# vvvwo/KSS-ICP

Hardware: AMD Instinct MI355X
Metric: icp_iterations_per_sec (higher is better)
Workload: dtype f32; 1 GPU; C2: one 100000x100000 uniform-sphere pair per GPU, 50 fixed ICP iterations + fitness pass per step (exact NN + cov reduce + host 3x3 SVD), R_z(10deg), jitter 1e-3; n_src=100000, n_tgt=100000, pairs_per_gpu=1, nn_engine=cell list + brute-force fallback, nn_arithmetic=reference (no fma)

## Files before the change

kss-icp_amd/csrc/kss_device.hpp:

```cpp
#pragma once
#include <hip/hip_runtime.h>

#include "kss_internal.hpp"

namespace kss {

template <bool FMA>
__device__ __forceinline__ float dist2(float sx, float sy, float sz, float tx, float ty, float tz) {
    const float dx = sx - tx, dy = sy - ty, dz = sz - tz;
    if constexpr (FMA) {
        return __builtin_fmaf(dx, dx, __builtin_fmaf(dy, dy, dz * dz));
    } else {
        return (dx * dx + dy * dy) + dz * dz;
    }
}

__device__ __forceinline__ int cell_coord(float v, float o, float inv_h, int g) {
    int c = (int)floorf((v - o) * inv_h);
    c = c < 0 ? 0 : c;
    return c >= g ? g - 1 : c;
}

__device__ __forceinline__ double wave_sum(double v) {
#pragma unroll
// ... 110 lines not shown
    v = 0.0;
    if (threadIdx.x < NSUMS)
        for (int gg = 0; gg < G; ++gg) v += shg[gg][threadIdx.x];
    return *s_ok != 0;
}

__device__ __forceinline__ void pub_put(unsigned long long* pub, int64_t slot, double v, unsigned long long seq, unsigned torn_xor = 0u) {
    const unsigned long long b = (unsigned long long)__double_as_longlong(v);
    u32x4 o;
    o.x = (unsigned)b; o.y = (unsigned)(b >> 32); o.z = (unsigned)seq; o.w = kss_mix3(o.x, o.y, o.z);
    o.x ^= torn_xor;
    unsigned long long* dst = pub + 2 * slot;
    asm volatile("global_store_dwordx4 %0, %1, off sc0 sc1" ::"v"(dst), "v"(o) : "memory");
}

constexpr int PASS_BS = 512;
constexpr int PASS_FG = PASS_BS / NSUMS;

template <typename F>
__device__ __forceinline__ double dpp_f64(double x, F f) {
    const int lo = f(__double2loint(x)), hi = f(__double2hiint(x));
    return __hiloint2double(hi, lo);
}
__device__ __forceinline__ double xor8(double x) { return dpp_f64(x, [](int v) { return __builtin_amdgcn_mov_dpp(v, 0x128, 0xf, 0xf, false); }); }
__device__ __forceinline__ double xor4(double x) {
    return dpp_f64(x, [](int v) {
        int r = __builtin_amdgcn_mov_dpp(v, 0x104, 0xf, 0x5, false);
        return __builtin_amdgcn_update_dpp(r, v, 0x114, 0xf, 0xa, false);
    });
}
__device__ __forceinline__ double xor2(double x) { return dpp_f64(x, [](int v) { return __builtin_amdgcn_mov_dpp(v, 0x4e, 0xf, 0xf, false); }); }
__device__ __forceinline__ double xor1(double x) { return dpp_f64(x, [](int v) { return __builtin_amdgcn_mov_dpp(v, 0xb1, 0xf, 0xf, false); }); }

__device__ __forceinline__ double level32(double a, double b) {
    unsigned alo = (unsigned)__double2loint(a), ahi = (unsigned)__double2hiint(a), blo = (unsigned)__double2loint(b), bhi = (unsigned)__double2hiint(b);
    asm volatile("s_nop 1\n\tv_permlane32_swap_b32 %0, %1\n\ts_nop 1" : "+v"(alo), "+v"(blo));
    asm volatile("s_nop 1\n\tv_permlane32_swap_b32 %0, %1\n\ts_nop 1" : "+v"(ahi), "+v"(bhi));
    return __hiloint2double((int)ahi, (int)alo) + __hiloint2double((int)bhi, (int)blo);
}
__device__ __forceinline__ double level16(double a, double b) {
    unsigned alo = (unsigned)__double2loint(a), ahi = (unsigned)__double2hiint(a), blo = (unsigned)__double2loint(b), bhi = (unsigned)__double2hiint(b);
    asm volatile("s_nop 1\n\tv_permlane16_swap_b32 %0, %1\n\ts_nop 1" : "+v"(alo), "+v"(blo));
    asm volatile("s_nop 1\n\tv_permlane16_swap_b32 %0, %1\n\ts_nop 1" : "+v"(ahi), "+v"(bhi));
    return __hiloint2double((int)ahi, (int)alo) + __hiloint2double((int)bhi, (int)blo);
}
__device__ __forceinline__ double tree_low4(double x) {
    x += xor8(x); x += xor4(x); x += xor2(x); x += xor1(x);
    return x;
}

__device__ __forceinline__ void wave_tree16(double (&v)[16]) {
#pragma unroll
    for (int j = 0; j < 8; ++j) v[j] = level32(v[j], v[j + 8]);
#pragma unroll
    for (int j = 0; j < 4; ++j) v[j] = level16(v[j], v[j + 4]);
#pragma unroll
    for (int j = 0; j < 4; ++j) v[j] = tree_low4(v[j]);
}
__device__ __forceinline__ double wave_tree2(double a, double b) {
    double x = level32(a, b);
    x = level16(x, x);
    return tree_low4(x);
}

__device__ __forceinline__ void accumulate_corr(double (&acc)[NSUMS], float px, float py, float pz,
                                                float qx, float qy, float qz, float d2f, double max_d2) {
    const double d2 = (double)d2f;
    acc[17] += d2;
    acc[18] += sqrt(d2);
    if (!(d2 > max_d2)) {
        const double p[3] = {(double)px, (double)py, (double)pz};
        const double q[3] = {(double)qx, (double)qy, (double)qz};
        acc[0] += 1.0;
#pragma unroll
        for (int k = 0; k < 3; ++k) { acc[1 + k] += p[k]; acc[4 + k] += q[k]; }
#pragma unroll
        for (int k = 0; k < 3; ++k)
#pragma unroll
            for (int l = 0; l < 3; ++l) acc[7 + 3 * k + l] += p[k] * q[l];
        acc[16] += d2;
    }
}


}
```

kss-icp_amd/csrc/kss_grid.hip:

```cpp
#pragma clang fp contract(off)

#include <hip/hip_runtime.h>

#include <cstring>

#include <rocprim/rocprim.hpp>

#include <cstdlib>

#include "kss_internal.hpp"
#include "kss_device.hpp"

namespace kss {

__global__ __launch_bounds__(256) void grid_count2_kernel(const float4* __restrict__ tgt, int nt, int nbt, const float4* __restrict__ src, int ns,
                                                          GridParams gp, int32_t* __restrict__ counts, int32_t* __restrict__ slot) {
    const bool is_src = (int)blockIdx.x >= nbt;
    const int i = ((int)blockIdx.x - (is_src ? nbt : 0)) * 256 + (int)threadIdx.x;
    if (i >= (is_src ? ns : nt)) return;
    const float4 p = is_src ? src[i] : tgt[i];
    const int cx = cell_coord(p.x, gp.ox, gp.inv_h, gp.gx), cy = cell_coord(p.y, gp.oy, gp.inv_h, gp.gy),
              cz = cell_coord(p.z, gp.oz, gp.inv_h, gp.gz);
    slot[(is_src ? nt : 0) + i] = atomicAdd(&counts[(is_src ? gp.gx * gp.gy * gp.gz : 0) + (cz * gp.gy + cy) * gp.gx + cx], 1);
}
// ... 294 lines not shown
        if (t == 4) continue;
        const float g2 = ey2[t % 3] + ez2[t / 3];
        const bool need = ok[t] && !(rho < g2 * 0.999999f);
        const bool left = !(rho < (g2 + exl2) * 0.999999f), right = !(rho < (g2 + exr2) * 0.999999f);
        const int lo = left ? s0[t] : s1[t];
        const int hi = right ? s3[t] : s2[t];
        const bool take = need && hi > lo;
        rowq[min(nrow, 7)][threadIdx.x] = make_int2(lo, hi);
        nrow += take ? 1 : 0;
        total += take ? hi - lo : 0;
    }
    int cur = 0, end = 0, nxt = 0;
    if (nrow > 0) { const int2 v = rowq[0][threadIdx.x]; cur = v.x; end = v.y; nxt = 1; }
    for (int e = 0; e < total; e += U) {
        int at[U];
#pragma unroll
        for (int j = 0; j < U; ++j) {
            at[j] = min(cur, end - 1);
            ++cur;
            if (cur >= end && nxt < nrow) { const int2 v = rowq[nxt][threadIdx.x]; cur = v.x; end = v.y; ++nxt; }
        }
        float4 pt[U];
#pragma unroll
        for (int j = 0; j < U; ++j) pt[j] = sorted[at[j]];
#pragma unroll
        for (int j = 0; j < U; ++j) {
            const unsigned long long kk = point_key<FMA>(pt[j], qx, qy, qz);
            if (kk < key) { key = kk; kpos = at[j]; }
            const float dd = e + j < total ? __uint_as_float((unsigned)(kk >> 32)) : __builtin_inff();
            m2 = __builtin_amdgcn_fmed3f(m1, m2, dd);
            m1 = fminf(m1, dd);
        }
    }
    return n4 + total;
}

__device__ __forceinline__ void row_range(const GridParams& gp, const int32_t* __restrict__ cell_start, float qx, float qy, float qz,
                                          int cx, int cy, int cz, float rho, int t, int& lo, int& hi) {
    lo = hi = 0;
    const int tz = t / 3, ty = t - 3 * tz;
    const int z = cz + tz - 1, y = cy + ty - 1;
    if (!(t >= 0 && t < 9 && z >= 0 && z < gp.gz && y >= 0 && y < gp.gy)) return;
    const int4u v = *(const int4u*)(cell_start + (z * gp.gy + y) * gp.gx + cx - 1);
    const int s0 = cx > 0 ? v.x : v.y, s1 = v.y, s2 = v.z, s3 = cx + 1 < gp.gx ? v.w : v.z;
    const float exl = fmaxf((qx - (gp.ox + (float)cx * gp.h)) - gp.eps, 0.f), exr = fmaxf(((gp.ox + (float)(cx + 1) * gp.h) - qx) - gp.eps, 0.f);
    const float eyl = fmaxf((qy - (gp.oy + (float)cy * gp.h)) - gp.eps, 0.f), eyr = fmaxf(((gp.oy + (float)(cy + 1) * gp.h) - qy) - gp.eps, 0.f);
    const float ezl = fmaxf((qz - (gp.oz + (float)cz * gp.h)) - gp.eps, 0.f), ezr = fmaxf(((gp.oz + (float)(cz + 1) * gp.h) - qz) - gp.eps, 0.f);
    const float ey2 = ty == 0 ? eyl * eyl : ty == 2 ? eyr * eyr : 0.f, ez2 = tz == 0 ? ezl * ezl : tz == 2 ? ezr * ezr : 0.f;
    const float g2 = ey2 + ez2;
    if (rho < g2 * 0.999999f) return;
    const bool left = !(rho < (g2 + exl * exl) * 0.999999f), right = !(rho < (g2 + exr * exr) * 0.999999f);
    lo = left ? s0 : s1;
    hi = right ? s3 : s2;
    if (hi < lo) hi = lo;
}

template <bool FMA, int U, bool TWO>
__device__ __forceinline__ void row_walk(const GridParams& gp, const int32_t* __restrict__ cell_start, const float4* __restrict__ sorted,
                                         float qx, float qy, float qz, int cx, int cy, int cz, float rho, int t0, int t1,
                                         unsigned long long& key, int& kpos, float& m1, float& m2) {
    m1 = __builtin_inff();
    m2 = __builtin_inff();
    int lo0, hi0, lo1 = 0, hi1 = 0;
    row_range(gp, cell_start, qx, qy, qz, cx, cy, cz, rho, t0, lo0, hi0);
    if constexpr (TWO) row_range(gp, cell_start, qx, qy, qz, cx, cy, cz, rho, t1, lo1, hi1);
    const int n0 = hi0 - lo0, total = n0 + (hi1 - lo1);
    const int last = hi1 > lo1 ? hi1 - 1 : hi0 - 1;
    for (int e = 0; e < total; e += U) {
        int at[U];
        float4 pt[U];
#pragma unroll
        for (int j = 0; j < U; ++j) {
            const int f = e + j;
            if constexpr (TWO) at[j] = f >= total ? last : f < n0 ? lo0 + f : lo1 + (f - n0);
            else at[j] = min(lo0 + f, hi0 - 1);
        }
#pragma unroll
        for (int j = 0; j < U; ++j) pt[j] = sorted[at[j]];
#pragma unroll
        for (int j = 0; j < U; ++j) {
            const unsigned long long kk = point_key<FMA>(pt[j], qx, qy, qz);
            if (kk < key) { key = kk; kpos = at[j]; }
            const float dd = e + j < total ? __uint_as_float((unsigned)(kk >> 32)) : __builtin_inff();
            m2 = __builtin_amdgcn_fmed3f(m1, m2, dd);
            m1 = fminf(m1, dd);
        }
    }
}

__global__ __launch_bounds__(256) void grid_rank_fix_kernel(const float4* __restrict__ tmp, int n, GridParams gp,
                                                            const int32_t* __restrict__ start , int shift,
                                                            float4* __restrict__ out) {
    const int j = blockIdx.x * blockDim.x + threadIdx.x;
    if (j >= n) return;
    const float4 p = tmp[j];
    const int cx = cell_coord(p.x, gp.ox, gp.inv_h, gp.gx), cy = cell_coord(p.y, gp.oy, gp.inv_h, gp.gy),
              cz = cell_coord(p.z, gp.oz, gp.inv_h, gp.gz);
    const int c = (cz * gp.gy + cy) * gp.gx + cx;
    const int lo = start[c] - shift, hi = start[c + 1] - shift;
    const int me = __float_as_int(p.w);
    int rank = 0;
    for (int k = lo; k < hi; ++k) rank += __float_as_int(tmp[k].w) < me ? 1 : 0;
    out[lo + rank] = p;
}

void launch_grid_build_pair(hipStream_t st, const float4* d_tgt, int nt, float4* d_src, int ns, const GridParams& gp, int32_t* d_counts,
                            int32_t* d_slot, int32_t* d_start, int32_t* d_block_sums, float4* d_sorted, float4* d_tmp) {
    const int ncells = gp.gx * gp.gy * gp.gz;
    const int nbt = (nt + 255) / 256, nbs = (ns + 255) / 256;
    hipLaunchKernelGGL(grid_count2_kernel, dim3(nbt + nbs), dim3(256), 0, st, d_tgt, nt, nbt, (const float4*)d_src, ns, gp, d_counts, d_slot);
    launch_scan(st, d_counts, 2 * ncells, d_start, d_block_sums, true);
    hipLaunchKernelGGL(grid_scatter2_kernel, dim3(nbt + nbs), dim3(256), 0, st, d_tgt, nt, nbt, (const float4*)d_src, ns, gp, (const int32_t*)d_slot,
                       (const int32_t*)d_start, d_sorted, d_tmp);
    hipLaunchKernelGGL(grid_rank_fix_kernel, dim3(nbs), dim3(256), 0, st, (const float4*)d_tmp, ns, gp, (const int32_t*)d_start + ncells, nt,
                       d_src);
}

struct SkipOut {
    unsigned long long key;
    int kpos;
    float rho;
    float acc;
    bool walker;
};
template <bool FMA>
__device__ __forceinline__ SkipOut skip_test(bool qok, float qx, float qy, float qz, float pold_x, float pold_y, float pold_z, const float4& prevp,
                                             const float2& st, bool chained_k, float skin_frac, float h) {
    SkipOut o;
    o.key = ~0ull; o.kpos = -1; o.rho = __builtin_inff(); o.acc = 0.f; o.walker = false;
    if (!qok) return o;
    o.walker = true;
    if (__float_as_uint(prevp.w) != ~0u) {
        o.key = point_key<FMA>(prevp, qx, qy, qz);
        o.kpos = -2;
        const float d0 = __uint_as_float((unsigned)(o.key >> 32));
        const float mx = qx - pold_x, my = qy - pold_y, mz = qz - pold_z;
        const float moved = __builtin_amdgcn_sqrtf((mx * mx + my * my) + mz * mz);
        const float acc = (st.y + moved) * 1.00001f;
        const float room = st.x - acc;
        if (chained_k && skin_frac >= 0.f && room > 1e-7f && (room * room) * 0.99999f > d0) {
            o.walker = false;
            o.acc = acc;
        } else {
            const float skin = fmaxf(skin_frac, 0.f) * h, grown = __builtin_amdgcn_sqrtf(d0) + skin;
            o.rho = !chained_k || moved * 4.f <= skin ? fmaxf(d0, grown * grown) : d0;
        }
    }
    return o;
}

template <bool FULL>
__device__ __forceinline__ void wave_row(bool have, bool kept, bool fell_back, float qx, float qy, float qz, const float4& win, double d2d, double* shw_row) {
    const int lane = threadIdx.x & 63;
    double col[16];
    {
        const double px = kept ? (double)qx : 0.0, py = kept ? (double)qy : 0.0, pz = kept ? (double)qz : 0.0;
        const double tx = kept ? (double)win.x : 0.0, ty = kept ? (double)win.y : 0.0, tz = kept ? (double)win.z : 0.0;
        col[0] = px; col[1] = py; col[2] = pz; col[3] = tx; col[4] = ty; col[5] = tz;
        col[6] = px * tx; col[7] = px * ty; col[8] = px * tz;
        col[9] = py * tx; col[10] = py * ty; col[11] = py * tz;
        col[12] = pz * tx; col[13] = pz * ty; col[14] = pz * tz;
        col[15] = kept ? d2d : 0.0;
    }
    wave_tree16(col);
    const unsigned long long mk = __builtin_amdgcn_ballot_w64(kept), mf = __builtin_amdgcn_ballot_w64(fell_back);
    double extra = 0.0;
    if constexpr (FULL) extra = wave_tree2(d2d, have ? sqrt(d2d) : 0.0);
    if ((lane & 15) == 0) {
        const int q = lane >> 4;
#pragma unroll
        for (int j = 0; j < 4; ++j) shw_row[1 + 4 * q + j] = col[j];
        if (lane == 0) {
            shw_row[0] = (double)__builtin_popcountll(mk);
            shw_row[NSUMS - 1] = (double)__builtin_popcountll(mf);
            shw_row[17] = extra;
        }
        if (lane == 32) shw_row[18] = extra;
    }
}

template <bool FMA, bool BATCH, int WQ, int NT, int U, bool FIRST = false>
__device__ __forceinline__ void serve_walkers(const PassArgs& a, const GridPairDev& pr, const int32_t* __restrict__ cs,
                                              const float4* __restrict__ sorted, int w, int nwalk, int2 (*rowq)[WQ],
                                              unsigned (*s_ent)[PASS_BS], const unsigned short* s_wl) {
#define KSS_STAMP(k) do { if (a.stamps && threadIdx.x == 0) a.stamps[(size_t)blockIdx.x * 16 + (k)] = __builtin_amdgcn_s_memrealtime(); } while (0)
    enum { WK_X, WK_Y, WK_Z, WK_IDX, WK_D2, WK_R, WK_POS, WK_FL = WK_POS, WK_COLS };
    const GridParams& gp = pr.gp;
    const int lane = threadIdx.x & 63;
    const bool row16 = 16 * nwalk <= NT, row8 = BATCH && !row16 && 8 * nwalk <= NT, rows = row16 || row8;
    const int L = row16 ? 16 : row8 ? 8 : 4 * nwalk <= WQ ? 4 : 1;
    const int nserve = rows ? NT : (WQ < NT ? WQ : NT);
    for (int rb = 0; rb < nwalk; rb += nserve / L)
    if ((int)threadIdx.x < nserve && (int)(threadIdx.x & ~63u) < (nwalk - rb) * L) {
        const int sub = (int)threadIdx.x & (L - 1);
        const int wj = rb + (L == 16 ? (int)threadIdx.x >> 4 : L == 8 ? (int)threadIdx.x >> 3 : L == 4 ? (int)threadIdx.x >> 2 : (int)threadIdx.x);
        const bool wk = wj < nwalk;
        const unsigned rowmask = L == 1 ? 0x1ffu : sub == 0 ? 0x105u : sub == 1 ? 0x050u : sub == 2 ? 0x082u : 0x028u;
        float wx = 0.f, wy = 0.f, wz = 0.f, wrho = __builtin_inff(), bnew = 0.f;
        unsigned long long wkey = ~0ull;
        int wpos = -1, owner = 0, evl = 0, rfin = 0;
        bool done = true, wfell = false;
        if (wk) {
            owner = (int)s_wl[wj];
            wx = __uint_as_float(s_ent[WK_X][owner]); wy = __uint_as_float(s_ent[WK_Y][owner]); wz = __uint_as_float(s_ent[WK_Z][owner]);
            wkey = ((unsigned long long)s_ent[WK_D2][owner] << 32) | (unsigned long long)s_ent[WK_IDX][owner];
            wpos = (int)s_ent[WK_POS][owner];
            wrho = __uint_as_float(s_ent[WK_R][owner]);
            done = false;
        }
        if (wk) {
            const int cx = cell_coord(wx, gp.ox, gp.inv_h, gp.gx), cy = cell_coord(wy, gp.oy, gp.inv_h, gp.gy),
                      cz = cell_coord(wz, gp.oz, gp.inv_h, gp.gz);
            KSS_STAMP(5);
            float m1, m2;
            if (row16) row_walk<FMA, U, false>(gp, cs, sorted, wx, wy, wz, cx, cy, cz, wrho, sub < 9 ? sub : -1, -1, wkey, wpos, m1, m2);
            else if (BATCH && row8) row_walk<FMA, U, true>(gp, cs, sorted, wx, wy, wz, cx, cy, cz, wrho, sub, sub == 0 ? 8 : -1, wkey, wpos, m1, m2);
            else if (FIRST && L == 1) evl = block_walk_first<FMA, WQ, U>(gp, cs, sorted, wx, wy, wz, cx, cy, cz, wrho, a.skin, rowq, wkey, wpos, m1, m2);
            else evl = block_walk<FMA, WQ, U>(gp, cs, sorted, wx, wy, wz, cx, cy, cz, wrho, rowmask, rowq, wkey, wpos, m1, m2);
            if (L > 1) {
#define KSS_GROUP_MERGE(X)                                                                                                          \
do {                                                                                                                            \
    const unsigned olo = (unsigned)X((int)(unsigned)wkey), ohi = (unsigned)X((int)(unsigned)(wkey >> 32));                      \
    const int opos = X(wpos);                                                                                                   \
    const float o1 = __int_as_float(X(__float_as_int(m1))), o2 = __int_as_float(X(__float_as_int(m2)));                         \
    const unsigned long long okey = ((unsigned long long)ohi << 32) | olo;                                                      \
    if (okey < wkey) { wkey = okey; wpos = opos; }                                                                            \
    m2 = fminf(fmaxf(m1, o1), fminf(m2, o2));                                \
    m1 = fminf(m1, o1);                                                                                                         \
} while (0)
                auto x1 = [](int v) { return __builtin_amdgcn_update_dpp(0, v, 0xb1, 0xf, 0xf, false); };
                auto x2 = [](int v) { return __builtin_amdgcn_update_dpp(0, v, 0x4e, 0xf, 0xf, false); };
                auto x4 = [](int v) { const int r = __builtin_amdgcn_update_dpp(v, v, 0x104, 0xf, 0x5, false); return __builtin_amdgcn_update_dpp(r, v, 0x114, 0xf, 0xa, false); };
                auto x8 = [](int v) { return __builtin_amdgcn_update_dpp(0, v, 0x128, 0xf, 0xf, false); };
                KSS_GROUP_MERGE(x1);
                KSS_GROUP_MERGE(x2);
                if (L >= 8) KSS_GROUP_MERGE(x4);
                if (L == 16) KSS_GROUP_MERGE(x8);
#undef KSS_GROUP_MERGE
            }
            float face2 = __builtin_inff();
            for (int r = 1; r <= gp.rcap; ++r) {
                if (r > 1) {
                    const int wd = 2 * r + 1;
                    const int x0 = max(cx - r, 0), x1 = min(cx + r, gp.gx - 1);
                    for (int t = 0; t < wd * wd; ++t) {
                        const int dz = t / wd - r, dy = t % wd - r;
                        const int z = cz + dz, y = cy + dy;
                        if (z < 0 || z >= gp.gz || y < 0 || y >= gp.gy) continue;
                        const int row = (z * gp.gy + y) * gp.gx;
                        if (dz == -r || dz == r || dy == -r || dy == r) {
                            scan_range<FMA>(sorted, cs[row + x0], cs[row + x1 + 1], wx, wy, wz, wkey, wpos);
                        } else {
                            if (cx - r >= 0) scan_range<FMA>(sorted, cs[row + cx - r], cs[row + cx - r + 1], wx, wy, wz, wkey, wpos);
                            if (cx + r < gp.gx) scan_range<FMA>(sorted, cs[row + cx + r], cs[row + cx + r + 1], wx, wy, wz, wkey, wpos);
                        }
                    }
                }
                const float best = __uint_as_float((unsigned)(wkey >> 32));
                float b = __builtin_inff();
                if (cx - r > 0) b = fminf(b, wx - (gp.ox + (float)(cx - r) * gp.h));
                if (cx + r < gp.gx - 1) b = fminf(b, (gp.ox + (float)(cx + r + 1) * gp.h) - wx);
                if (cy - r > 0) b = fminf(b, wy - (gp.oy + (float)(cy - r) * gp.h));
                if (cy + r < gp.gy - 1) b = fminf(b, (gp.oy + (float)(cy + r + 1) * gp.h) - wy);
                if (cz - r > 0) b = fminf(b, wz - (gp.oz + (float)(cz - r) * gp.h));
                if (cz + r < gp.gz - 1) b = fminf(b, (gp.oz + (float)(cz + r + 1) * gp.h) - wz);
                const float bs = b - gp.eps;
                if (b == __builtin_inff()) done = true;
                else if (bs > 0.f && best < bs * bs * 0.999999f) { done = true; face2 = bs * bs; }
                if (done) { rfin = r; break; }
            }
            if (done && rfin == 1 && wkey != ~0ull)
                bnew = fminf(__builtin_amdgcn_sqrtf(fminf(fminf(m2, wrho), face2) * 0.99999f) * 0.999999f, 1e30f);
        }
        if constexpr (BATCH) {
            if (__builtin_amdgcn_ballot_w64(!done) != 0ull) {
                const float4* __restrict__ tp = a.tgt4 + pr.tgt_base;
                for (int j = 0; j < pr.tgt_n; ++j) {
                    const float4 q = tp[j];
                    const float dx = wx - q.x, dy = wy - q.y, dz = wz - q.z;
                    float d;
                    if constexpr (FMA) d = __builtin_fmaf(dx, dx, __builtin_fmaf(dy, dy, dz * dz));
                    else d = (dx * dx + dy * dy) + dz * dz;
                    const unsigned long long kk = ((unsigned long long)__float_as_uint(d) << 32) | (unsigned long long)(unsigned)j;
                    if (!done && kk < wkey) { wkey = kk; wpos = -1; }
                }
                wfell = !done;
                done = true;
            }
        }
        if (wk && sub == 0) {
            bool whave = false;
            float4 ww = make_float4(0.f, 0.f, 0.f, 0.f);
            const int io = pr.src_base + (w - pr.row_base) * PASS_BS + owner;
            if (done) {
                whave = wkey != ~0ull;
                if (whave) ww = wpos >= 0 ? sorted[wpos] : wpos == -2 ? a.nn_win[io] : a.tgt4[pr.tgt_base + (int)(unsigned)(wkey & 0xffffffffull)];
            } else {
                a.keys[io] = ~0ull;
                const int ls = atomicAdd(a.list_count, 1);
                a.list[ls] = io;
                wfell = true;
            }
            a.nn_win[io] = make_float4(ww.x, ww.y, ww.z, __uint_as_float(whave ? (unsigned)wkey : ~0u));
            a.nn_state[io] = make_float2(wfell ? 0.f : bnew, 0.f);
            s_ent[WK_X][owner] = __float_as_uint(ww.x); s_ent[WK_Y][owner] = __float_as_uint(ww.y); s_ent[WK_Z][owner] = __float_as_uint(ww.z);
            s_ent[WK_IDX][owner] = (unsigned)wkey; s_ent[WK_D2][owner] = (unsigned)(wkey >> 32);
            s_ent[WK_FL][owner] = (whave ? 1u : 0u) | (wfell ? 2u : 0u);
            s_ent[WK_R][owner] = __float_as_uint(wfell ? 0.f : bnew);
        }
        KSS_STAMP(8);
        if (a.stamps) {
            int evs = evl, mx = evl;
#pragma unroll
            for (int m = 32; m > 0; m >>= 1) { evs += __shfl_xor(evs, m, 64); mx = max(mx, __shfl_xor(mx, m, 64)); }
            if (lane == 0) {
                atomicAdd(&a.stamps[(size_t)blockIdx.x * 16 + 10], (unsigned long long)evs);
                atomicAdd(&a.stamps[(size_t)blockIdx.x * 16 + 11], (unsigned long long)(((mx + 7) / 8) * 8 * 64));
            }
        }
    }
#undef KSS_STAMP
}

#ifndef KSS_BATCH_WAVES
#define KSS_BATCH_WAVES 6
#endif
#ifndef KSS_SINGLE_WAVES
#define KSS_SINGLE_WAVES 1
#endif
template <bool FMA, bool FULL, bool BATCH, bool SEARCH, bool CHAIN, bool FIRST = false>
__global__ __launch_bounds__(PASS_BS, BATCH ? KSS_BATCH_WAVES : KSS_SINGLE_WAVES) void grid_pass_kernel(const PassArgs a) {
    static_assert(!CHAIN || (!BATCH && SEARCH), "chained launches: single pair, search passes");
    static_assert(!FIRST || (!BATCH && SEARCH && !CHAIN), "the first pass: single pair, a plain search launch");
#define KSS_STAMP(k) do { if (a.stamps && threadIdx.x == 0) a.stamps[(size_t)blockIdx.x * 16 + (k)] = __builtin_amdgcn_s_memrealtime(); } while (0)
    KSS_STAMP(0);
    constexpr int BS = PASS_BS;
    const int per_xcd = (int)gridDim.x / 8;
    const int w = ((int)blockIdx.x % 8) * per_xcd + (int)blockIdx.x / 8;
    if (w >= a.total_rows) return;
    int pi = 0;
    if constexpr (BATCH) pi = a.row_pair[w];
    const GridPairDev pr = BATCH ? a.pairs[pi] : a.pair0;
    PairState ps = a.ps0;
    if constexpr (BATCH) {
        ps = a.state[pi];
        if (!ps.active) return;
    }
    const GridParams& gp = pr.gp;
    const int32_t* __restrict__ cs = a.cell_start + pr.cell_base;
    const float4* __restrict__ sorted = a.sorted;
    constexpr int WQ = FIRST ? BS : 256;
    __shared__ int2 rowq[9][WQ];
    __shared__ double shw[BS / 64][NSUMS];
    __shared__ int s_last;
    __shared__ int sh_ps[16];
    __shared__ int s_nwalk;
    __shared__ unsigned s_ent[7][BS];
    __shared__ unsigned short s_wl[BS];
    enum { WK_X, WK_Y, WK_Z, WK_IDX, WK_D2, WK_R, WK_POS, WK_FL = WK_POS, WK_COLS };
    static_assert(sizeof(PairState) == 64, "the gated launch reads the transform record as 16 dwords");
    double (*shf)[NSUMS] = reinterpret_cast<double (*)[NSUMS]>(&rowq[0][0]);
    static_assert(sizeof(double) * PASS_FG * NSUMS <= sizeof(int2) * 9 * WQ, "shf must fit inside rowq");

    const int local = (w - pr.row_base) * BS + (int)threadIdx.x;
    const bool valid = local < pr.src_n;
    const int i = pr.src_base + local;
    const int lane = threadIdx.x & 63, wave = threadIdx.x >> 6;
    bool have = false, fell_back = false;
    float qx = 0.f, qy = 0.f, qz = 0.f, d2 = 0.f;
    float4 win = make_float4(0.f, 0.f, 0.f, 0.f);
    float4 p = make_float4(0.f, 0.f, 0.f, 0.f), prevp = make_float4(0.f, 0.f, 0.f, __uint_as_float(~0u));
    float2 st = make_float2(0.f, 0.f);
    if (valid) {
        p = SEARCH ? a.src_in[i] : a.src_out[i];
        if (!SEARCH || a.use_prev) { prevp = a.nn_win[i]; st = a.nn_state[i]; }
    }
    for (int step = 0;; ++step) {
    const bool last_step = !CHAIN || step + 1 >= a.chain_len;
    const unsigned long long seq_k = a.seq + (unsigned long long)step;
    const int gate_k = a.gate_seq != 0 ? a.gate_seq + step : 0;
    unsigned int* const gate_ptr = a.gate_dev + 32 * ((a.gate_slot + step) & 1);
    float4* const src_out_k = (step & 1) ? a.src_alt : a.src_out;
    const bool last_known = a.chained == 2 && ps.pad[0] > 0;
    const bool chained_k = step > 0 || a.chained == 1 || last_known;
    const bool has_prev = __float_as_uint(prevp.w) != ~0u;
    if constexpr (SEARCH) {
        __syncthreads();
        if (threadIdx.x == 0) s_nwalk = 0;
        __syncthreads();
    }
    KSS_STAMP(13);
    if constexpr (!BATCH && SEARCH) {
        if (gate_k != 0) {
            typedef unsigned int u32x4 __attribute__((ext_vector_type(4)));
            if (a.state && w == 0 && threadIdx.x < 16) {
                const int* w32 = reinterpret_cast<const int*>(a.state);
                int v = 0, n = 0;
                bool ok = true;
                for (;;) {
                    v = __hip_atomic_load(w32 + threadIdx.x, __ATOMIC_RELAXED, __HIP_MEMORY_SCOPE_SYSTEM);
                    if (__shfl(v, 15, 64) == gate_k) break;
                    __builtin_amdgcn_s_sleep(1);
                    if (++n > a.gate_polls / 2) { ok = false; break; }
                }
                if (ok) {
                    const int g = threadIdx.x;
                    const int w0 = __shfl(v, min(3 * g, 15), 64), w1 = __shfl(v, min(3 * g + 1, 15), 64), w2 = __shfl(v, min(3 * g + 2, 15), 64);
                    if (g < 5) {
                        u32x4 o;
                        o.x = (unsigned)w0; o.y = (unsigned)w1; o.z = (unsigned)w2; o.w = (unsigned)gate_k + kss_mix3(o.x, o.y, o.z);
                        unsigned int* dst = gate_ptr + 4 * g;
                        asm volatile("global_store_dwordx4 %0, %1, off sc1" ::"v"(dst), "v"(o) : "memory");
                    }
                }
            }
            if (threadIdx.x < 8) {
// ... 3 lines not shown
                bool ok = true;
                for (;;) {
                    asm volatile("global_load_dwordx4 %0, %1, off sc0 sc1\n\ts_waitcnt vmcnt(0)" : "=&v"(v) : "v"(src) : "memory");
                    if (__builtin_amdgcn_ballot_w64(v.w - kss_mix3(v.x, v.y, v.z) == (unsigned)gate_k) == 0xffull) break;
                    __builtin_amdgcn_s_sleep(1);
                    if (++n > a.gate_polls) { ok = false; break; }
                }
                if (threadIdx.x < 5) { sh_ps[3 * threadIdx.x] = (int)v.x; sh_ps[3 * threadIdx.x + 1] = (int)v.y; sh_ps[3 * threadIdx.x + 2] = (int)v.z; }
                if (threadIdx.x == 0) { sh_ps[15] = gate_k; s_last = ok ? 1 : 0; }
            }
            __syncthreads();
            if (!s_last) return;
            int* d32 = reinterpret_cast<int*>(&ps);
#pragma unroll
            for (int k = 0; k < 16; ++k) d32[k] = sh_ps[k];
            if (ps.pad[0] != 0) return;
            __syncthreads();
            KSS_STAMP(9);
        }
    }
    unsigned long long key = ~0ull;
    float pold_x = p.x, pold_y = p.y, pold_z = p.z;
    if (SEARCH && last_known && valid) {
        const float4 pl = (ps.pad[0] == 1 ? a.src_last0 : a.src_last1)[i];
        pold_x = pl.x; pold_y = pl.y; pold_z = pl.z;
    }
    if (valid) {
        if constexpr (SEARCH) {
            if (ps.apply) {
                const float x = p.x, y = p.y, z = p.z;
                p.x = ((ps.m[0] * x + ps.m[1] * y) + ps.m[2] * z) + ps.m[3];
                p.y = ((ps.m[4] * x + ps.m[5] * y) + ps.m[6] * z) + ps.m[7];
                p.z = ((ps.m[8] * x + ps.m[9] * y) + ps.m[10] * z) + ps.m[11];
            }
            src_out_k[i] = p;
        }
        qx = p.x; qy = p.y; qz = p.z;
        const bool qok = (qx - qx) == 0.f && (qy - qy) == 0.f && (qz - qz) == 0.f;
        if constexpr (!SEARCH) {
            if (has_prev) {
                win = prevp;
                key = point_key<FMA>(win, qx, qy, qz);
            } else if (qok) {
                key = a.keys[i];
                if (key != ~0ull) win = a.tgt4[pr.tgt_base + (int)(unsigned)(key & 0xffffffffull)];
            }
            have = key != ~0ull;
        }
    }
    if constexpr (SEARCH) {
        bool walker = false;
        float acc_keep = 0.f;
        {
            const bool qok = valid && (qx - qx) == 0.f && (qy - qy) == 0.f && (qz - qz) == 0.f;
            const SkipOut so = skip_test<FMA>(qok, qx, qy, qz, pold_x, pold_y, pold_z, prevp, st, chained_k, a.skin, gp.h);
            walker = so.walker;
            key = so.key;
            acc_keep = so.acc;
            unsigned fl = 0u;
            if (qok && !walker) {
                fl = 1u;
                a.nn_state[i] = make_float2(st.x, so.acc);
            } else if (valid && !qok) {
                a.nn_win[i] = make_float4(0.f, 0.f, 0.f, __uint_as_float(~0u));
                a.nn_state[i] = make_float2(0.f, 0.f);
            }
            const float4 c4 = walker ? make_float4(qx, qy, qz, 0.f) : prevp;
            s_ent[WK_X][threadIdx.x] = __float_as_uint(c4.x); s_ent[WK_Y][threadIdx.x] = __float_as_uint(c4.y); s_ent[WK_Z][threadIdx.x] = __float_as_uint(c4.z);
            s_ent[WK_IDX][threadIdx.x] = (unsigned)key; s_ent[WK_D2][threadIdx.x] = (unsigned)(key >> 32);
            s_ent[WK_POS][threadIdx.x] = walker ? (unsigned)so.kpos : fl;
            s_ent[WK_R][threadIdx.x] = __float_as_uint(so.rho);
        }
        const unsigned long long wm = __builtin_amdgcn_ballot_w64(walker);
        if (wm != 0ull) {
            int base = 0;
            if (lane == 0) base = atomicAdd(&s_nwalk, (int)__builtin_popcountll(wm));
            base = __builtin_amdgcn_readfirstlane(base);
            if (walker) s_wl[base + (int)__builtin_amdgcn_mbcnt_hi((unsigned)(wm >> 32), __builtin_amdgcn_mbcnt_lo((unsigned)wm, 0u))] = (unsigned short)threadIdx.x;
        }
        KSS_STAMP(14);
        __syncthreads();
        const int nwalk = s_nwalk;
        if (a.stamps && threadIdx.x == 0) a.stamps[(size_t)blockIdx.x * 16 + 12] = (unsigned long long)nwalk;
        serve_walkers<FMA, BATCH, WQ, BS, BATCH ? 4 : 8, FIRST>(a, pr, cs, sorted, w, nwalk, rowq, s_ent, s_wl);
        KSS_STAMP(15);
        __syncthreads();
        {
            const unsigned fl = s_ent[WK_FL][threadIdx.x];
            have = (fl & 1u) != 0u; fell_back = (fl & 2u) != 0u;
            win = make_float4(__uint_as_float(s_ent[WK_X][threadIdx.x]), __uint_as_float(s_ent[WK_Y][threadIdx.x]), __uint_as_float(s_ent[WK_Z][threadIdx.x]), 0.f);
            key = ((unsigned long long)s_ent[WK_D2][threadIdx.x] << 32) | (unsigned long long)s_ent[WK_IDX][threadIdx.x];
            if (CHAIN && !last_step) {
                if (walker) {
                    prevp = make_float4(win.x, win.y, win.z, __uint_as_float(have ? (unsigned)key : ~0u));
                    st = make_float2(__uint_as_float(s_ent[WK_R][threadIdx.x]), 0.f);
                } else if (have) {
                    st.y = acc_keep;
                } else {
                    prevp.w = __uint_as_float(~0u);
                    st = make_float2(0.f, 0.f);
                }
            }
        }
        if constexpr (BATCH) {
            p = make_float4(0.f, 0.f, 0.f, 0.f);
            if (valid) p = src_out_k[i];
            qx = p.x; qy = p.y; qz = p.z;
        }
    }
    if (valid && have) {
        d2 = __uint_as_float((unsigned)(key >> 32));
        const int oi = __float_as_int(p.w);
        if (a.idx_out) a.idx_out[oi] = (int)(unsigned)(key & 0xffffffffull);
        if (a.d2_out) a.d2_out[oi] = d2;
    }
    KSS_STAMP(1);

    const double d2d = have ? (double)d2 : 0.0;
    const bool kept = have && !(d2d > a.max_d2);
    wave_row<FULL>(have, kept, fell_back, qx, qy, qz, win, d2d, shw[wave]);
    __syncthreads();
    double r = 0.0;
    if (threadIdx.x < NSUMS)
#pragma unroll
        for (int ww = 0; ww < BS / 64; ++ww) r += shw[ww][threadIdx.x];
    KSS_STAMP(2);

    double v = 0.0 + r;
    if (pr.n_rows > 1) {
        Granule* const rows = a.rows + (int64_t)pr.row_base * NSUMS;
        if (threadIdx.x < NSUMS) row_put(rows + (int64_t)(w - pr.row_base) * NSUMS, threadIdx.x, r, seq_k);
        KSS_STAMP(3);
        if (w != pr.row_base || a.defer_pairs) {
            if (last_step) return;
            continue;
        }
        if (!rows_total<PASS_FG>(rows, pr.n_rows, seq_k, 1 << 20, shf, &s_last, v)) return;
    }
    if (threadIdx.x < NSUMS) {
        if (!FULL && (threadIdx.x == 17 || threadIdx.x == 18)) v = 0.0;
        const int64_t slot = (int64_t)pi * NSUMS + threadIdx.x;
        if (a.test_torn && threadIdx.x == 5) {
            pub_put(a.pub, slot, v, seq_k, 0x00100000u);
            asm volatile("s_waitcnt vmcnt(0)" ::: "memory");
            for (int k = 0; k < 400; ++k) __builtin_amdgcn_s_sleep(64);
        }
        pub_put(a.pub, slot, v, seq_k);
        KSS_STAMP(4);
    }
    if (last_step) break;
    }
#undef KSS_STAMP
}

#ifndef KSS_BATCH2_WAVES
#define KSS_BATCH2_WAVES 5
#endif
template <bool FMA, bool FULL, int WQ>
__global__ __launch_bounds__(256, KSS_BATCH2_WAVES) void gridb_pass_kernel(const PassArgs a) {
#define KSS_STAMP(k) do { if (a.stamps && threadIdx.x == 0) a.stamps[(size_t)blockIdx.x * 16 + (k)] = __builtin_amdgcn_s_memrealtime(); } while (0)
    KSS_STAMP(0);
    constexpr int BS = PASS_BS, NT = 256, SPL = BS / NT;
    static_assert(SPL == 2 && WQ <= NT, "two sources per lane");
    const int per_xcd = (int)gridDim.x / 8;
    const int w = ((int)blockIdx.x % 8) * per_xcd + (int)blockIdx.x / 8;
    if (w >= a.total_rows) return;
    const int pi = a.row_pair[w];
// ... 372 lines not shown
        float4 p[GB_U];
#pragma unroll
        for (int u = 0; u < GB_U; ++u) p[u] = sp[min(k0 + u * GB_THREADS, pr.src_n - 1)];
#pragma unroll
        for (int u = 0; u < GB_U; ++u) {
            const int k = k0 + u * GB_THREADS;
            if (k < pr.src_n) {
                const int pos = cnt.add1(cell_of(p[u]));
                p[u].w = __int_as_float(pr.src_base + k);
                tmp[pos] = p[u];
            }
        }
    }
    __syncthreads();
    float4* out = src_out + pr.src_base;
    for (int j0 = tid; j0 < pr.src_n; j0 += GB_THREADS * GB_U) {
        float4 p[GB_U];
#pragma unroll
        for (int u = 0; u < GB_U; ++u) p[u] = tmp[min(j0 + u * GB_THREADS, pr.src_n - 1)];
#pragma unroll
        for (int u = 0; u < GB_U; ++u) {
            if (j0 + u * GB_THREADS >= pr.src_n) continue;
            const int c = cell_of(p[u]);
            const int lo = c > 0 ? cnt.get(c - 1) : 0, hi = cnt.get(c);
            const int me = __float_as_int(p[u].w);
            int rank = 0;
            for (int k = lo; k < hi; ++k) rank += __float_as_int(tmp[k].w) < me ? 1 : 0;
            out[lo + rank] = p[u];
        }
    }
}

bool launch_gridb_build_lds(hipStream_t st, const float4* d_tgt4, float4* d_src, float4* d_tmp, const GridPairDev* d_pairs, int npairs,
                            int32_t* d_cell_start, float4* d_sorted, int max_cells, bool half) {
    const size_t bytes = half ? (size_t)((max_cells + 1) / 2) * 4 : (size_t)max_cells * 4;
    {
        const int most = GB_MAX_CELLS * 4;
        const void* fn = half ? reinterpret_cast<const void*>(&gridb_build_pair_kernel<true>) : reinterpret_cast<const void*>(&gridb_build_pair_kernel<false>);
        if (hipFuncSetAttribute(fn, hipFuncAttributeMaxDynamicSharedMemorySize, most) != hipSuccess) { (void)hipGetLastError(); return false; }
    }
    if (half)
        hipLaunchKernelGGL(gridb_build_pair_kernel<true>, dim3(npairs), dim3(GB_THREADS), bytes, st, d_tgt4, (const float4*)d_src, d_tmp, d_src, d_pairs,
                           d_cell_start, d_sorted);
    else
        hipLaunchKernelGGL(gridb_build_pair_kernel<false>, dim3(npairs), dim3(GB_THREADS), bytes, st, d_tgt4, (const float4*)d_src, d_tmp, d_src, d_pairs,
                           d_cell_start, d_sorted);
    return true;
}

__global__ __launch_bounds__(256) void grid_stats_kernel(const float4* __restrict__ src, int ns, GridParams gp,
                                                         const int32_t* __restrict__ cell_start, unsigned long long* __restrict__ out) {
    const int i = blockIdx.x * blockDim.x + threadIdx.x;
    unsigned long long ev = 0, occ = 0;
    if (i < ns) {
        const float4 p = src[i];
        const int cx = cell_coord(p.x, gp.ox, gp.inv_h, gp.gx), cy = cell_coord(p.y, gp.oy, gp.inv_h, gp.gy),
                  cz = cell_coord(p.z, gp.oz, gp.inv_h, gp.gz);
        const int x0 = max(cx - 1, 0), x1 = min(cx + 1, gp.gx - 1);
        for (int t = 0; t < 9; ++t) {
            const int z = cz + t / 3 - 1, y = cy + t % 3 - 1;
            if (z < 0 || z >= gp.gz || y < 0 || y >= gp.gy) continue;
            const int row = (z * gp.gy + y) * gp.gx;
            ev += (unsigned long long)(cell_start[row + x1 + 1] - cell_start[row + x0]);
        }
    }
    const int ncells = gp.gx * gp.gy * gp.gz;
    for (int c = blockIdx.x * blockDim.x + threadIdx.x; c < ncells; c += gridDim.x * blockDim.x)
        occ += cell_start[c + 1] > cell_start[c] ? 1 : 0;
    atomicAdd(&out[0], ev);
    atomicAdd(&out[1], occ);
}

void launch_grid_stats(hipStream_t st, const float4* d_src, int ns, const GridParams& gp, const int32_t* d_cell_start,
                       unsigned long long* d_out) {
    hipLaunchKernelGGL(grid_stats_kernel, dim3((ns + 255) / 256), dim3(256), 0, st, d_src, ns, gp, d_cell_start, d_out);
}

int grid_pass_blocks(int total_rows) { return (total_rows + 7) / 8 * 8; }

void launch_grid_pass(hipStream_t st, bool fma, bool full, bool batch, bool search, const PassArgs& a) {
    if (a.total_rows <= 0) return;
    const dim3 grid(grid_pass_blocks(a.total_rows)), block(PASS_BS);
    static const bool first_pass = getenv("KSS_FIRST_PASS") == nullptr || atoi(getenv("KSS_FIRST_PASS")) != 0;
#define KSS_PASS(F, U, B, S) hipLaunchKernelGGL((grid_pass_kernel<F, U, B, S, false>), grid, block, 0, st, a)
#define KSS_CHAIN(F, U) hipLaunchKernelGGL((grid_pass_kernel<F, U, false, true, true>), grid, block, 0, st, a)
    if (!search) {
        if (fma) KSS_PASS(true, true, false, false); else KSS_PASS(false, true, false, false);
    } else if (batch) {
        static const bool old_form = getenv("KSS_BATCH_OLD") != nullptr;
        if (old_form) {
            if (fma) { if (full) KSS_PASS(true, true, true, true); else KSS_PASS(true, false, true, true); }
            else     { if (full) KSS_PASS(false, true, true, true); else KSS_PASS(false, false, true, true); }
        } else {
            const dim3 block2(256);
#define KSS_PASSB(F, U, Q) hipLaunchKernelGGL((gridb_pass_kernel<F, U, Q>), grid, block2, 0, st, a)
            if (!a.use_prev) {
                if (fma) { if (full) KSS_PASSB(true, true, 256); else KSS_PASSB(true, false, 256); }
                else     { if (full) KSS_PASSB(false, true, 256); else KSS_PASSB(false, false, 256); }
            } else {
                if (fma) { if (full) KSS_PASSB(true, true, 128); else KSS_PASSB(true, false, 128); }
                else     { if (full) KSS_PASSB(false, true, 128); else KSS_PASSB(false, false, 128); }
            }
#undef KSS_PASSB
        }
        if (a.defer_pairs) hipLaunchKernelGGL(gridb_finalize_kernel, dim3(a.defer_pairs), dim3(256), 0, st, a, full ? 1 : 0);
    } else if (a.chain_len > 1) {
        if (fma) { if (full) KSS_CHAIN(true, true); else KSS_CHAIN(true, false); }
        else     { if (full) KSS_CHAIN(false, true); else KSS_CHAIN(false, false); }
    } else if (first_pass && !a.use_prev) {
#define KSS_FIRST(F, U) hipLaunchKernelGGL((grid_pass_kernel<F, U, false, true, false, true>), grid, block, 0, st, a)
        if (fma) { if (full) KSS_FIRST(true, true); else KSS_FIRST(true, false); }
        else     { if (full) KSS_FIRST(false, true); else KSS_FIRST(false, false); }
#undef KSS_FIRST
    } else {
        if (fma) { if (full) KSS_PASS(true, true, false, true); else KSS_PASS(true, false, false, true); }
        else     { if (full) KSS_PASS(false, true, false, true); else KSS_PASS(false, false, false, true); }
    }
#undef KSS_PASS
#undef KSS_CHAIN
}

}
```

Measured before the change: 85640 iterations/s.

## Split cell-row scans into fixed slices balanced across 16-lane walker groups

Adds a row-split walk mode for single-pair search passes. Each 16-lane group computes a DPP prefix sum over its rows' slice counts, writes (start, length) slices of 8 points into shared memory, and redistributes them so each lane scans one slice instead of one whole cell row. This is meant to remove load imbalance where long rows serialize a walker while other lanes sit idle. When a group has more than 16 slices it falls back to per-row scanning. It is enabled by default through an environment variable, also applies to chained launches, and adds LDS writes plus a wave barrier.

```diff
diff --git a/kss-icp_amd/csrc/kss_device.hpp b/kss-icp_amd/csrc/kss_device.hpp
--- a/kss-icp_amd/csrc/kss_device.hpp
+++ b/kss-icp_amd/csrc/kss_device.hpp
@@ -216,5 +216,14 @@
     }
 }
 
-
-}
+constexpr int ROW_SPLIT_U = 8, ROW_SPLIT_LANES = 16;
+__host__ __device__ __forceinline__ int row_split_slices(int n) { return (n + ROW_SPLIT_U - 1) / ROW_SPLIT_U; }
+__host__ __device__ __forceinline__ bool row_split_put(int lo, int n, int p, int total, int2* table) {
+    if (total > ROW_SPLIT_LANES) return false;
+    for (int j = 0, left = n; left > 0; ++j, left -= ROW_SPLIT_U)
+        table[p + j] = make_int2(lo + ROW_SPLIT_U * j, left < ROW_SPLIT_U ? left : ROW_SPLIT_U);
+    return true;
+}
+
+
+}
diff --git a/kss-icp_amd/csrc/kss_grid.hip b/kss-icp_amd/csrc/kss_grid.hip
--- a/kss-icp_amd/csrc/kss_grid.hip
+++ b/kss-icp_amd/csrc/kss_grid.hip
@@ -400,6 +400,52 @@
             const unsigned long long kk = point_key<FMA>(pt[j], qx, qy, qz);
             if (kk < key) { key = kk; kpos = at[j]; }
             const float dd = e + j < total ? __uint_as_float((unsigned)(kk >> 32)) : __builtin_inff();
+            m2 = __builtin_amdgcn_fmed3f(m1, m2, dd);
+            m1 = fminf(m1, dd);
+        }
+    }
+}
+
+template <bool FMA, int U>
+__device__ __forceinline__ void row_walk_split(const GridParams& gp, const int32_t* __restrict__ cell_start, const float4* __restrict__ sorted,
+                                               float qx, float qy, float qz, int cx, int cy, int cz, float rho, int sub, int2* tab,
+                                               unsigned long long& key, int& kpos, float& m1, float& m2) {
+    static_assert(U == ROW_SPLIT_U, "one slice = one step");
+    m1 = __builtin_inff();
+    m2 = __builtin_inff();
+    int lo, hi;
+    row_range(gp, cell_start, qx, qy, qz, cx, cy, cz, rho, sub < 9 ? sub : -1, lo, hi);
+    int n = hi - lo;
+    const int ch = row_split_slices(n);
+    int inc = ch;
+    inc += __builtin_amdgcn_update_dpp(0, inc, 0x111, 0xf, 0xf, true);
+    inc += __builtin_amdgcn_update_dpp(0, inc, 0x112, 0xf, 0xf, true);
+    inc += __builtin_amdgcn_update_dpp(0, inc, 0x114, 0xf, 0xf, true);
+    inc += __builtin_amdgcn_update_dpp(0, inc, 0x118, 0xf, 0xf, true);
+    const int t0 = __builtin_amdgcn_readlane(inc, 15), t1 = __builtin_amdgcn_readlane(inc, 31), t2 = __builtin_amdgcn_readlane(inc, 47),
+              t3 = __builtin_amdgcn_readlane(inc, 63);
+    const int g = ((int)threadIdx.x & 63) >> 4;
+    const int total = g == 0 ? t0 : g == 1 ? t1 : g == 2 ? t2 : t3;
+    if (row_split_put(lo, n, inc - ch, total, tab)) {
+        asm volatile("s_waitcnt lgkmcnt(0)" ::: "memory");
+        __builtin_amdgcn_wave_barrier();
+        const int2 e = tab[sub];
+        lo = e.x;
+        n = sub < total ? e.y : 0;
+    }
+    const int last = lo + n - 1;
+    for (int e = 0; e < n; e += U) {
+        int at[U];
+        float4 pt[U];
+#pragma unroll
+        for (int j = 0; j < U; ++j) at[j] = min(lo + e + j, last);
+#pragma unroll
+        for (int j = 0; j < U; ++j) pt[j] = sorted[at[j]];
+#pragma unroll
+        for (int j = 0; j < U; ++j) {
+            const unsigned long long kk = point_key<FMA>(pt[j], qx, qy, qz);
+            if (kk < key) { key = kk; kpos = at[j]; }
+            const float dd = e + j < n ? __uint_as_float((unsigned)(kk >> 32)) : __builtin_inff();
             m2 = __builtin_amdgcn_fmed3f(m1, m2, dd);
             m1 = fminf(m1, dd);
         }
@@ -497,7 +543,7 @@
     }
 }
 
-template <bool FMA, bool BATCH, int WQ, int NT, int U, bool FIRST = false>
+template <bool FMA, bool BATCH, int WQ, int NT, int U, bool FIRST = false, bool SPLIT = false>
 __device__ __forceinline__ void serve_walkers(const PassArgs& a, const GridPairDev& pr, const int32_t* __restrict__ cs,
                                               const float4* __restrict__ sorted, int w, int nwalk, int2 (*rowq)[WQ],
                                               unsigned (*s_ent)[PASS_BS], const unsigned short* s_wl) {
@@ -531,6 +577,10 @@
                       cz = cell_coord(wz, gp.oz, gp.inv_h, gp.gz);
             KSS_STAMP(5);
             float m1, m2;
+            if constexpr (SPLIT) {
+                if (row16) row_walk_split<FMA, U>(gp, cs, sorted, wx, wy, wz, cx, cy, cz, wrho, sub, &rowq[0][0] + ((int)threadIdx.x & ~15), wkey, wpos, m1, m2);
+                else evl = block_walk<FMA, WQ, U>(gp, cs, sorted, wx, wy, wz, cx, cy, cz, wrho, rowmask, rowq, wkey, wpos, m1, m2);
+            } else
             if (row16) row_walk<FMA, U, false>(gp, cs, sorted, wx, wy, wz, cx, cy, cz, wrho, sub < 9 ? sub : -1, -1, wkey, wpos, m1, m2);
             else if (BATCH && row8) row_walk<FMA, U, true>(gp, cs, sorted, wx, wy, wz, cx, cy, cz, wrho, sub, sub == 0 ? 8 : -1, wkey, wpos, m1, m2);
             else if (FIRST && L == 1) evl = block_walk_first<FMA, WQ, U>(gp, cs, sorted, wx, wy, wz, cx, cy, cz, wrho, a.skin, rowq, wkey, wpos, m1, m2);
@@ -646,10 +696,11 @@
 #ifndef KSS_SINGLE_WAVES
 #define KSS_SINGLE_WAVES 1
 #endif
-template <bool FMA, bool FULL, bool BATCH, bool SEARCH, bool CHAIN, bool FIRST = false>
+template <bool FMA, bool FULL, bool BATCH, bool SEARCH, bool CHAIN, bool FIRST = false, bool SPLIT = false>
 __global__ __launch_bounds__(PASS_BS, BATCH ? KSS_BATCH_WAVES : KSS_SINGLE_WAVES) void grid_pass_kernel(const PassArgs a) {
     static_assert(!CHAIN || (!BATCH && SEARCH), "chained launches: single pair, search passes");
     static_assert(!FIRST || (!BATCH && SEARCH && !CHAIN), "the first pass: single pair, a plain search launch");
+    static_assert(!SPLIT || (!BATCH && SEARCH && !FIRST), "the row split: single pair, search passes after the first");
 #define KSS_STAMP(k) do { if (a.stamps && threadIdx.x == 0) a.stamps[(size_t)blockIdx.x * 16 + (k)] = __builtin_amdgcn_s_memrealtime(); } while (0)
     KSS_STAMP(0);
     constexpr int BS = PASS_BS;
@@ -819,7 +870,7 @@
         __syncthreads();
         const int nwalk = s_nwalk;
         if (a.stamps && threadIdx.x == 0) a.stamps[(size_t)blockIdx.x * 16 + 12] = (unsigned long long)nwalk;
-        serve_walkers<FMA, BATCH, WQ, BS, BATCH ? 4 : 8, FIRST>(a, pr, cs, sorted, w, nwalk, rowq, s_ent, s_wl);
+        serve_walkers<FMA, BATCH, WQ, BS, BATCH ? 4 : 8, FIRST, SPLIT>(a, pr, cs, sorted, w, nwalk, rowq, s_ent, s_wl);
         KSS_STAMP(15);
         __syncthreads();
         {
@@ -1358,8 +1409,11 @@
     if (a.total_rows <= 0) return;
     const dim3 grid(grid_pass_blocks(a.total_rows)), block(PASS_BS);
     static const bool first_pass = getenv("KSS_FIRST_PASS") == nullptr || atoi(getenv("KSS_FIRST_PASS")) != 0;
+    static const bool row_split = getenv("KSS_ROW_SPLIT") == nullptr || atoi(getenv("KSS_ROW_SPLIT")) != 0;
 #define KSS_PASS(F, U, B, S) hipLaunchKernelGGL((grid_pass_kernel<F, U, B, S, false>), grid, block, 0, st, a)
-#define KSS_CHAIN(F, U) hipLaunchKernelGGL((grid_pass_kernel<F, U, false, true, true>), grid, block, 0, st, a)
+#define KSS_SEARCH1(F, U, C) do { if (row_split) hipLaunchKernelGGL((grid_pass_kernel<F, U, false, true, C, false, true>), grid, block, 0, st, a); \
+                                  else hipLaunchKernelGGL((grid_pass_kernel<F, U, false, true, C, false, false>), grid, block, 0, st, a); } while (0)
+#define KSS_CHAIN(F, U) KSS_SEARCH1(F, U, true)
     if (!search) {
         if (fma) KSS_PASS(true, true, false, false); else KSS_PASS(false, true, false, false);
     } else if (batch) {
@@ -1389,10 +1443,11 @@
         else     { if (full) KSS_FIRST(false, true); else KSS_FIRST(false, false); }
 #undef KSS_FIRST
     } else {
-        if (fma) { if (full) KSS_PASS(true, true, false, true); else KSS_PASS(true, false, false, true); }
-        else     { if (full) KSS_PASS(false, true, false, true); else KSS_PASS(false, false, false, true); }
+        if (fma) { if (full) KSS_SEARCH1(true, true, false); else KSS_SEARCH1(true, false, false); }
+        else     { if (full) KSS_SEARCH1(false, true, false); else KSS_SEARCH1(false, false, false); }
     }
 #undef KSS_PASS
+#undef KSS_SEARCH1
 #undef KSS_CHAIN
 }
 
```

Result: no change. 86810 iterations/s (median of 6 runs) (+1.4%).
